# StavrosOrf/EV2Gym

Measured on AMD Instinct MI355X. Metric: env-steps/sec (envs x chargers x steps); % HBM roofline, higher is better.
Workload: dtype f64; 1 GPU; cfg2: V2GProfitPlusLoads, 50 chargers, 1 transformer, uniform[-1,1] actions; envs_per_gpu=4096, scenario_pool_per_gpu=32768, scenario_pool_order=sorted by busy window inside every window of envs_per_gpu scenarios, chargers=50, transformers=1, steps_per_episode=112, obs_dim=162, soc_log=True, launch=persistent, actor=none

## Files before the change

ev2gym_amd/csrc/ev2g_device.h:

```cpp
#pragma once
#include <hip/hip_runtime.h>
#include <stdint.h>

#define EV2G_BLOCK 256
#define EV2G_NQ 8

#include "ev2g_records.h"
typedef SessDyn PortDyn;

struct DevScn {
    int E;
    int M;
    int T, C, npc, P, R, D, ND, dt;
    int reward_kind, state_kind, flags, cost_kind;
    int n_lut;
    int G;
    int gs;
    int n_groups;
    double sixty_over_dt;
    double dt_over_60;
    const int *slot_port, *slot_cs, *slot_obs, *slot_tr;
    const int *cs_np, *cs_pbase, *slot_mask;
    const int *cs_slot0;
    int het;
// ... 854 lines not shown
    z = z ^ (z >> 31);
    return (double)(z >> 11) * (1.0 / 9007199254740992.0);
}

__global__ void ev2g_fill_uniform_kernel(double *dst, long long n, uint64_t seed, double lo, double hi) {
    for (long long i = blockIdx.x * (long long)blockDim.x + threadIdx.x; i < n; i += (long long)gridDim.x * blockDim.x)
        dst[i] = lo + (hi - lo) * ev2g_u01(seed, (uint64_t)i);
}

__device__ __forceinline__ double wave_sum(double v) {
    for (int d = 32; d > 0; d >>= 1) v += __shfl_xor(v, d, 64);
    return v;
}
__device__ __forceinline__ double wave_min(double v) {
    for (int d = 32; d > 0; d >>= 1) v = fmin(v, __shfl_xor(v, d, 64));
    return v;
}

__device__ __forceinline__ void port_sessions(const DevScn &s, const DevState &st, long long g, long long gs, int cur_step, int &first,
                                              int &last, bool &attached) {
    first = s.port_first[gs];
    last = first;
    attached = false;
    if (first < 0) return;
    const int2 w = make_int2(st.line[g].ta, st.line[g].td);
    const int cur = st.line[g].ss;
    if (cur < 0) {
        last = s.port_end[gs];
    } else {
        attached = (w.x <= cur_step);
        last = attached ? cur + 1 : cur;
    }
}

template <int EPWS> __device__ __forceinline__ double seg_sum(double v) {
    v += xor1_f64(v);
    v += xor2_f64(v);
    v += xor4_f64(v);
    v += dpp_mov_f64<0x128>(v);
    const int lo = __double2loint(v), hi = __double2hiint(v);
    const double r0 = __hiloint2double(__builtin_amdgcn_readlane(hi, 0), __builtin_amdgcn_readlane(lo, 0));
    const double r1 = __hiloint2double(__builtin_amdgcn_readlane(hi, 16), __builtin_amdgcn_readlane(lo, 16));
    const double r2 = __hiloint2double(__builtin_amdgcn_readlane(hi, 32), __builtin_amdgcn_readlane(lo, 32));
    const double r3 = __hiloint2double(__builtin_amdgcn_readlane(hi, 48), __builtin_amdgcn_readlane(lo, 48));
    if (EPWS == 1) return (r0 + r1) + (r2 + r3);
    return (threadIdx.x < 32) ? r0 + r1 : r2 + r3;
}
template <int EPWS> __device__ __forceinline__ double seg_min(double v) {
    v = fmin(v, xor1_f64(v));
    v = fmin(v, xor2_f64(v));
    v = fmin(v, xor4_f64(v));
    v = fmin(v, dpp_mov_f64<0x128>(v));
    const int lo = __double2loint(v), hi = __double2hiint(v);
    const double r0 = __hiloint2double(__builtin_amdgcn_readlane(hi, 0), __builtin_amdgcn_readlane(lo, 0));
    const double r1 = __hiloint2double(__builtin_amdgcn_readlane(hi, 16), __builtin_amdgcn_readlane(lo, 16));
    const double r2 = __hiloint2double(__builtin_amdgcn_readlane(hi, 32), __builtin_amdgcn_readlane(lo, 32));
    const double r3 = __hiloint2double(__builtin_amdgcn_readlane(hi, 48), __builtin_amdgcn_readlane(lo, 48));
    if (EPWS == 1) return fmin(fmin(r0, r1), fmin(r2, r3));
    return (threadIdx.x < 32) ? fmin(r0, r1) : fmin(r2, r3);
}
template <int EPWS> __device__ __forceinline__ bool seg_all(bool p) {
    const unsigned long long m = __ballot(p);
    if (EPWS == 1) return m == ~0ull;
    return (threadIdx.x < 32) ? ((unsigned)m == 0xffffffffu) : ((unsigned)(m >> 32) == 0xffffffffu);
}

struct StatsView {
    int T, C, R, P, dt;
    const double *setpoint;
    const int *scn_sess, *scn_sess_end, *ss_slot, *ss_tarr, *ss_tdep;
    const double *ss_B, *ss_afap;
    const int *cs_served;
    const double *cs_sat_sum, *hist, *env_acc, *sess_final_cap, *sess_abs_e, *soc_log;
    const PortLine *line;
};
__device__ __forceinline__ StatsView ev2g_stats_view(const DevScn &s, const DevState &st, const double *ss_afap) {
    return StatsView{s.T, s.C, s.R, s.P, s.dt, s.setpoint, s.scn_sess, s.scn_sess_end, s.ss_slot, s.ss_tarr, s.ss_tdep, s.ss_B, ss_afap,
                     st.cs_served, st.cs_sat_sum, st.hist, st.env_acc, st.sess_final_cap, st.sess_abs_e, st.soc_log, st.line};
}

#define EV2G_STATS_NK 40
#define EV2G_STATS_TB 8
#define EV2G_STATS_LK 16

template <int EPWS, int NK, int LK>
__device__ __forceinline__ void ev2g_env_stats(const StatsView &sv, int e, bool e_valid, int scn, int lane, int cur_step, double *__restrict__ out,
                                               double *l_keep, int lslot) {
    constexpr int W = 64 / EPWS;
    const int T = sv.T, C = sv.C, R = sv.R, P = sv.P;
    double served = 0.0, sat = 0.0, nsat = 0.0;
    for (int c = lane; c < C; c += W) {
        const int n = sv.cs_served[(long long)e * C + c];
        served += n;
        if (n > 0) { sat += sv.cs_sat_sum[(long long)e * C + c] / n; nsat += 1.0; }
    }
    served = seg_sum<EPWS>(served); sat = seg_sum<EPWS>(sat); nsat = seg_sum<EPWS>(nsat);
    double over = 0.0, te = 0.0, ete = 0.0, ptv = 0.0;
    for (int t = lane; t < T; t += W) {
        const bool past = t < cur_step;
        if (past) for (int r = 0; r < R; r++) over += sv.hist[EV2G_HIST(e, t, T, R) + 2 + r];
        const double sp = sv.setpoint[(long long)scn * T + t], u = past ? sv.hist[EV2G_HIST(e, t, T, R)] : 0.0;
        const double d = sp - u;
        te += d * d;
        ete += fabs(d);
        if (u > sp) ptv += u - sp;
    }
    over = seg_sum<EPWS>(over); te = seg_sum<EPWS>(te); ete = seg_sum<EPWS>(ete); ptv = seg_sum<EPWS>(ptv);
    ete *= (double)sv.dt / 60.0;
    if (lane == 0 && e_valid) {
        double *o = out + (long long)e * 17;
        o[0] = served;
        o[4] = (nsat > 0.0) ? sat / nsat : NAN;
        o[5] = ptv;
        o[6] = te;
        o[7] = ete;
        o[12] = over;
    }
    const double e0 = 7.543e6, e1 = 23.75e6, e2 = 6976, z0 = 7.348e-3, z1 = 3.667, z2 = 7.6e-4, z3 = 4.081e-3;
    const double b_cap_ah = 2.05, b_cap_kwh = 78, d_dist = 15000, b_age = 2 * 365, G_ = 0.186;
    const double theta = 298.15, kk = 0.8263, v_min = 3.3324;
    const double k_arrh = exp(-e2 / theta), k_age = pow(b_age, 0.25);
    const double Q_acc = 2 * (b_age * (d_dist / 365) * G_ * b_cap_ah) / b_cap_kwh, k_qacc = pow(Q_acc, 0.5);
    const bool log_soc = sv.soc_log != nullptr;
    double sum = 0.0, mn = INFINITY, cnt = 0.0, deg_cal = 0.0, deg_cyc = 0.0;
    double vkeep[2];
    int nkeep = 0;
    const int d0 = sv.scn_sess[scn], d1 = sv.scn_sess_end[scn];
    for (int k0 = d0; k0 < d1; k0 += W) {
        const int k = min(k0 + lane, d1 - 1);
        const bool has = k0 + lane < d1;
        const int q = sv.ss_slot[k], ta = sv.ss_tarr[k], td = sv.ss_tdep[k];
        const double B = sv.ss_B[k], afap = sv.ss_afap[k], fin_cap = sv.sess_final_cap[k];
        const double fin_abs = log_soc ? sv.sess_abs_e[k] : 0.0;
        const long long g = (long long)e * P + q;
        const bool spawned = has && ta <= cur_step;
        const bool live = td >= cur_step;
        const double l_cap = sv.line[g].cap, l_abs = sv.line[g].abse;
        const double capk = live ? l_cap : fin_cap;
        if (spawned) {
            const double v = capk / afap * 100.0;
            sum += v;
            mn = fmin(mn, v);
            cnt += 1.0;
            if (nkeep < 2) vkeep[nkeep] = v;
            nkeep++;
        }
        if (spawned) {
            if (log_soc) {
                const double *__restrict__ slog = sv.soc_log + (long long)e * T * P + q;
                const int tend = min(td, cur_step - 1);
                const double soc_f = capk / B;
                const double invB = 1.0 / B;
                double hs = 0.0, fs = 0.0;
                int n = 0, nf = 0;
                double xk[NK];
#pragma unroll
                for (int u = 0; u < NK; u++) xk[u] = slog[(long long)min(ta + u, tend) * P];
#pragma unroll
                for (int u = 0; u < NK; u++) {
                    if (ta + u <= tend) {
                        const double soc = fabs(xk[u]) * invB;
                        hs += soc; n++;
                        if (__double_as_longlong(xk[u]) >= 0) { fs += soc; nf++; }
                    }
                }
                for (int t = ta + NK; t <= tend; t += EV2G_STATS_TB) {
                    double x[EV2G_STATS_TB];
#pragma unroll
                    for (int u = 0; u < EV2G_STATS_TB; u++) x[u] = slog[(long long)min(t + u, tend) * P];
                    if (LK > 0 && t - ta - NK < LK) {
#pragma unroll
                        for (int u = 0; u < EV2G_STATS_TB; u++) l_keep[(t - ta - NK + u) * 64 + lslot] = x[u];
                    }
#pragma unroll
                    for (int u = 0; u < EV2G_STATS_TB; u++) {
                        if (t + u <= tend) {
                            const double soc = fabs(x[u]) * invB;
                            hs += soc; n++;
                            if (__double_as_longlong(x[u]) >= 0) { fs += soc; nf++; }
                        }
                    }
                }
                hs += soc_f; n++;
                fs += soc_f; nf++;
                const double avg_soc = hs / n, avg_f = fs / nf;
                double mad = 0.0;
#pragma unroll
                for (int u = 0; u < NK; u++)
                    if (ta + u <= tend && __double_as_longlong(xk[u]) >= 0) mad += fabs(avg_f - fabs(xk[u]) * invB);
                for (int t = ta + NK; t <= tend; t += EV2G_STATS_TB) {
                    double x[EV2G_STATS_TB];
                    if (LK > 0 && t - ta - NK < LK) {
#pragma unroll
                        for (int u = 0; u < EV2G_STATS_TB; u++) x[u] = l_keep[(t - ta - NK + u) * 64 + lslot];
                    } else {
#pragma unroll
                        for (int u = 0; u < EV2G_STATS_TB; u++) x[u] = slog[(long long)min(t + u, tend) * P];
                    }
#pragma unroll
                    for (int u = 0; u < EV2G_STATS_TB; u++)
                        if (t + u <= tend && __double_as_longlong(x[u]) >= 0) mad += fabs(avg_f - fabs(x[u]) * invB);
                }
                mad += fabs(avg_f - soc_f);
                const double delta_DoD = 2 * (mad / nf);
                const double T_sim = (td - ta + 1) * (double)sv.dt / (60 * 24);
                const double v_avg = v_min + kk * avg_soc;
                const double alpha = (e0 * v_avg - e1) * k_arrh;
                deg_cal += alpha * 0.75 * T_sim / k_age;
                const double v_half = v_min + kk * 0.5;
                const double beta = z0 * (v_half - z1) * (v_half - z1) + z2 + z3 * delta_DoD;
                const double abs_e = live ? l_abs : fin_abs;
                const double Q_sim = (abs_e / b_cap_kwh) * b_cap_ah;
                deg_cyc += beta * 0.5 * Q_sim / k_qacc;
            }
        }
    }
    sum = seg_sum<EPWS>(sum); cnt = seg_sum<EPWS>(cnt); mn = seg_min<EPWS>(mn);
    deg_cal = seg_sum<EPWS>(deg_cal); deg_cyc = seg_sum<EPWS>(deg_cyc);
    if (lane == 0 && e_valid) {
        const double *acc = sv.env_acc + (long long)e * 8;
        double *o = out + (long long)e * 17;
        o[1] = acc[1];
        o[2] = acc[2];
        o[3] = acc[3];
        o[11] = acc[4];
        o[13] = log_soc ? deg_cal + deg_cyc : NAN;
        o[14] = log_soc ? deg_cal : NAN;
        o[15] = log_soc ? deg_cyc : NAN;
        o[16] = acc[0];
    }
    double mean = NAN, sd = NAN, mnv = NAN;
    if (cnt > 0.0) {
        mean = sum / cnt;
        double var = 0.0;
        if (seg_all<EPWS>(nkeep <= 2)) {
            if (nkeep > 0) { const double v = vkeep[0] - mean; var += v * v; }
            if (nkeep > 1) { const double v = vkeep[1] - mean; var += v * v; }
        } else {
            for (int k = d0 + lane; k < d1; k += W) {
                const int ta = sv.ss_tarr[k];
                if (ta <= cur_step) {
                    const double capk = (sv.ss_tdep[k] >= cur_step) ? sv.line[(long long)e * P + sv.ss_slot[k]].cap : sv.sess_final_cap[k];
                    const double v = capk / sv.ss_afap[k] * 100.0 - mean;
                    var += v * v;
                }
            }
        }
        var = seg_sum<EPWS>(var);
        sd = sqrt(var / cnt);
        mnv = mn;
    }
    if (lane == 0 && e_valid) {
        double *o = out + (long long)e * 17;
        o[8] = mean;
        o[9] = sd;
        o[10] = mnv;
    }
}

template <int W>
__device__ __forceinline__ void ev2g_env_reset(const DevScn &s, const DevState &st, int e, int lane, int reset_off, double *__restrict__ r_obs,
                                               float *__restrict__ r_obs32) {
    const int T = s.T, C = s.C, R = s.R, P = s.P;
    const int scn_n = ev2g_scn(e, reset_off, s.M);
    const bool hfast = s.head_tab != nullptr && s.state_kind != 1 && 2 + s.head_nh <= 2 * W && (r_obs || r_obs32);
    double hrow0 = 0.0, hrow1 = 0.0;
    if (hfast) {
        const double *row = s.head_tab + (long long)scn_n * (T + 1) * s.head_nh;
        hrow0 = row[min(max(lane - 2, 0), s.head_nh - 1)];
        hrow1 = row[min(lane + W - 2, s.head_nh - 1)];
    }
    for (int q = lane; q < P; q += W) {
        const long long g = (long long)e * P + q, gs = (long long)scn_n * P + q;
        const int2 w = s.port_first_win[gs];
        st.line[g].ta = w.x; st.line[g].td = w.y; st.line[g].ss = s.port_first[gs]; st.line[g].cyc_lut = 0;
        st.line[g].cap = 0.0; st.line[g].tot = 0.0; st.line[g].prev = 0.0;
        st.port_energy[g] = 0.0; st.port_current[g] = 0.0;
        if (r_obs) { double *o = r_obs + (long long)e * s.D + s.slot_obs[q]; o[0] = 0.0; o[1] = 0.0; if (s.state_kind == 1) o[2] = 0.0; }
        if (r_obs32) { float *o = r_obs32 + (long long)e * s.D + s.slot_obs[q]; o[0] = 0.f; o[1] = 0.f; if (s.state_kind == 1) o[2] = 0.f; }
    }
    for (int c = lane; c < C; c += W) {
        const long long gc = (long long)e * C + c;
        st.cs_sat_sum[gc] = 0.0; st.cs_served[gc] = 0;
        if (st.cs_profits) { st.cs_profits[gc] = 0.0; st.cs_e_ch[gc] = 0.0; st.cs_e_dis[gc] = 0.0; st.cs_power_now[gc] = 0.0; st.cs_cur_now[gc] = 0.0; }
    }
    for (int i = lane; i < 8; i += W) st.env_acc[(long long)e * 8 + i] = 0.0;
    if (lane == 0) st.hist[EV2G_HIST(e, 0, T, R) + 1] = 0.0;
    for (int r = lane; r < R; r += W) st.tr_power_now[(long long)e * R + r] = 0.0;
    if (lane == 0) st.env_fault[e] = 0;
    if (hfast) {
        const int c0 = lane, c1 = lane + W, nc = 2 + s.head_nh;
        const double v0 = (c0 < 2) ? 0.0 : hrow0;
        if (r_obs) { double *o = r_obs + (long long)e * s.D; if (c0 < nc) o[c0] = v0; if (c1 < nc) o[c1] = hrow1; }
        if (r_obs32) { float *o = r_obs32 + (long long)e * s.D; if (c0 < nc) o[c0] = (float)v0; if (c1 < nc) o[c1] = (float)hrow1; }
    } else {
        if (r_obs) write_obs_env(s, r_obs + (long long)e * s.D, scn_n, 0, 0.0, lane, W);
        if (r_obs32) write_obs_env(s, r_obs32 + (long long)e * s.D, scn_n, 0, 0.0, lane, W);
    }
}

template <int EPWS, bool RESET = false>
__global__ void __launch_bounds__(64) ev2g_stats_kernel(DevScn s, DevState st, int scn_off,
                                                        const double *__restrict__ ss_afap, int cur_step,
                                                        double *__restrict__ out, int reset_off = 0, double *__restrict__ r_obs = nullptr,
                                                        float *__restrict__ r_obs32 = nullptr) {
    constexpr int W = 64 / EPWS;
    const int sub = threadIdx.x / W, lane = threadIdx.x - sub * W;
    const int e_raw = blockIdx.x * EPWS + sub;
    const bool e_valid = e_raw < s.E;
    const int e = e_valid ? e_raw : s.E - 1;
    const int scn = ev2g_scn(e, scn_off, s.M);
    extern __shared__ double l_keep[];
    ev2g_env_stats<EPWS, EV2G_STATS_NK, EV2G_STATS_LK>(ev2g_stats_view(s, st, ss_afap), e, e_valid, scn, lane, cur_step, out, l_keep, (int)threadIdx.x);
    if (RESET && e_valid) ev2g_env_reset<W>(s, st, e, lane, reset_off, r_obs, r_obs32);
}

template <int EPWS>
__global__ void __launch_bounds__(64) ev2g_copy_stats_reset_kernel(DevScn s, DevState st, const double *__restrict__ done_stats, double *__restrict__ out,
                                                                   int reset_off, double *__restrict__ r_obs, float *__restrict__ r_obs32) {
    constexpr int W = 64 / EPWS;
    const int sub = threadIdx.x / W, lane = threadIdx.x - sub * W;
    const int e = blockIdx.x * EPWS + sub;
    if (e >= s.E) return;
    for (int j = lane; j < 17; j += W) out[(long long)e * 17 + j] = done_stats[(long long)e * 17 + j];
    ev2g_env_reset<W>(s, st, e, lane, reset_off, r_obs, r_obs32);
}
```

ev2gym_amd/csrc/ev2g_host.hip:

```cpp
#include <hip/hip_runtime.h>

#include <algorithm>
#include <cmath>
#include <cstdio>
#include <cstring>
#include <array>
#include <map>
#include <string>
#include <utility>
#include <vector>

#include "../../include/ev2g.h"
#include "ev2g_device.h"
#include "ev2g_load_host.h"
#include "ev2g_route_host.h"
#include "ev2g_policy_host.h"
#include "ev2g_step_v2.h"
#include "ev2g_step_wave.h"
#include "ev2g_step_big.h"
#include "ev2g_mlp.h"
#include "ev2g_comm.h"
#include "ev2g_refill.h"
#include "ev2g_heuristic.h"
#include "ev2g_link.h"
// ... 2390 lines not shown
}

int ev2g_host_adam(float *theta, float *m, float *v, const float *g, int64_t n, int64_t t, double lr, double beta1, double beta2, double eps) {
    if (!theta || !m || !v || !g || n < 0 || t < 1) return fail(nullptr, EV2G_ERR_ARG, "ev2g_host_adam: null argument, n < 0 or t < 1");
    if (!std::isfinite(lr) || !(beta1 >= 0.0 && beta1 < 1.0) || !(beta2 >= 0.0 && beta2 < 1.0) || !(eps > 0.0))
        return fail(nullptr, EV2G_ERR_ARG, "ev2g_host_adam: lr must be finite, the betas in [0, 1), eps > 0");
    const AdamStep a = adam_step(lr, beta1, beta2, eps, (long long)t);
    for (int64_t i = 0; i < n; i++) ev2g_adam_elem(theta + i, m + i, v + i, g[i], a);
    return EV2G_OK;
}

int ev2g_host_ppo_head(const float *mean, const float *value, const float *actions, const float *log_std, const float *old_log_prob,
                       const float *advantages, const float *returns, int B, int P, const ev2g_ppo_config *cfg, float *d_mean, float *d_value,
                       float *d_log_std, float *stats) {
    if (!mean || !value || !actions || !log_std || !old_log_prob || !advantages || !returns || !cfg || !d_mean || !d_value || !d_log_std || !stats)
        return fail(nullptr, EV2G_ERR_ARG, "ev2g_host_ppo_head: null argument");
    if (B < 1 || P < 1) return fail(nullptr, EV2G_ERR_ARG, "ev2g_host_ppo_head: B and P must be positive");
    const bool norm = cfg->normalize_advantage && B > 1;
    double a_mean = 0.0, a_scale = 1.0;
    if (norm) {
        double s = 0.0;
        for (int i = 0; i < B; i++) s += (double)advantages[i];
        a_mean = s / B;
        s = 0.0;
        for (int i = 0; i < B; i++) { const double d = (double)advantages[i] - a_mean; s += d * d; }
        a_scale = 1.0 / (std::sqrt(s / (double)(B - 1)) + 1e-8);
    }
    std::vector<double> iv((size_t)P), dls((size_t)P, 0.0);
    for (int p = 0; p < P; p++) iv[(size_t)p] = std::exp(-2.0 * (double)log_std[p]);
    const double inv_b = 1.0 / (double)B;
    double sum[4] = {0.0, 0.0, 0.0, 0.0};
    for (int i = 0; i < B; i++) {
        const float *mu = mean + (size_t)i * P, *a = actions + (size_t)i * P;
        double q[8];
        for (int j = 0; j < 8; j++) q[j] = ev2g_ppo_lp_part(mu, a, log_std, iv.data(), P, j, 8);
        const float A = norm ? (float)(((double)advantages[i] - a_mean) * a_scale) : advantages[i];
        const PpoRow o = ev2g_ppo_head_row(ev2g_ppo_join8(q), old_log_prob[i], A, returns[i], value[i], (float)cfg->clip_range, (float)cfg->vf_coef, inv_b);
        d_value[i] = o.g_v;
        sum[0] += o.pol; sum[1] += o.vsq; sum[2] += o.kl; sum[3] += o.clipped;
        for (int p = 0; p < P; p++) {
            float dl;
            ev2g_ppo_head_port(a[p], mu[p], iv[(size_t)p], o.g_lp, d_mean + (size_t)i * P + p, &dl);
            dls[(size_t)p] += (double)dl;
        }
    }
    for (int p = 0; p < P; p++) d_log_std[p] = (float)(dls[(size_t)p] - cfg->ent_coef);
    ev2g_ppo_stats(sum, log_std, P, inv_b, (float)cfg->vf_coef, (float)cfg->ent_coef, stats);
    return EV2G_OK;
}

int ev2g_check_faults(ev2g_handle *h, int32_t *first_bad_env) {
    if (!h || !h->loaded) return fail(h, EV2G_ERR_STATE, "ev2g_check_faults: no scenarios loaded");
    (void)hipSetDevice(h->device);
    std::vector<int> f(h->E);
    HIPCHK(h, hipMemcpyAsync(f.data(), h->st.env_fault, sizeof(int) * h->E, hipMemcpyDeviceToHost, h->stream));
    HIPCHK(h, hipStreamSynchronize(h->stream));
    for (int e = 0; e < h->E; e++)
        if (f[e]) {
            if (first_bad_env) *first_bad_env = e;
            return fail(h, EV2G_ERR_OVERCURRENT, "charger over-current: sum of amps is higher than max charge current (ev_charger.py:203-205)");
        }
    return EV2G_OK;
}

static int launch_stats(ev2g_handle *h, double *stats, bool reset, double *obs, long long off, float *obs32 = nullptr) {
    (void)hipSetDevice(h->device);
    const bool copy = h->last.inl_stats && h->current_step == h->T;
    h->last_stats_route = copy ? 1 : 0;
    h->stats_reason = copy ? "" : h->last.inl_reason;
    if (copy && !reset) {
        HIPCHK(h, hipMemcpyAsync(stats, h->d_stats_inl, sizeof(double) * (size_t)h->E * EV2G_N_STATS, hipMemcpyDeviceToDevice, h->stream));
        return EV2G_OK;
    }

    const bool pair = stats_pair(h);
    const dim3 grid(pair ? (h->E + 1) / 2 : h->E);
    if (copy) {
        hipLaunchKernelGGL((ev2g_copy_stats_reset_kernel<1>), dim3(h->E), dim3(64), 0, h->stream, h->scn, h->st, (const double *)h->d_stats_inl, stats, (int)off, obs,
                           obs32 ? obs32 : (float *)h->extras.obs_f32);
        HIPCHK(h, hipGetLastError());
        return EV2G_OK;
    }
#define EV2G_STATS_LAUNCH(EPWS, RESET)                                                                                                    \
    hipLaunchKernelGGL((ev2g_stats_kernel<EPWS, RESET>), grid, dim3(64), (size_t)EV2G_STATS_LK * 64 * sizeof(double), h->stream, h->scn, h->st, (int)h->scn_off, (const double *)h->d_ss_afap, \
                       h->current_step, stats, (int)off, obs, RESET ? (obs32 ? obs32 : (float *)h->extras.obs_f32) : (float *)nullptr)
    if (pair) { if (reset) EV2G_STATS_LAUNCH(2, true); else EV2G_STATS_LAUNCH(2, false); }
    else { if (reset) EV2G_STATS_LAUNCH(1, true); else EV2G_STATS_LAUNCH(1, false); }
#undef EV2G_STATS_LAUNCH
    HIPCHK(h, hipGetLastError());
    return EV2G_OK;
}

int ev2g_get_stats(ev2g_handle *h, double *stats) {
    if (!h || !h->loaded) return fail(h, EV2G_ERR_STATE, "ev2g_get_stats: no scenarios loaded");
    if (!stats) return fail(h, EV2G_ERR_ARG, "ev2g_get_stats: null output");
    return launch_stats(h, stats, false, nullptr, 0);
}

static int stats_reset_impl(ev2g_handle *h, double *stats, double *obs, float *obs32, int64_t scenario_offset) {
    if (!h || !h->loaded) return fail(h, EV2G_ERR_STATE, "ev2g_get_stats_reset: no scenarios loaded");
    if (!stats) return fail(h, EV2G_ERR_ARG, "ev2g_get_stats_reset: null output");
    long long off = scenario_offset % (long long)h->scn.M;
    if (off < 0) off += h->scn.M;
    const int rc = launch_stats(h, stats, true, obs, off, obs32);
    if (rc) return rc;
    if (h->st.cs_power_hist) {
        HIPCHK(h, hipMemsetAsync(h->st.cs_power_hist, 0, sizeof(double) * (size_t)h->scn.T * h->scn.E * h->scn.C, h->stream));
        HIPCHK(h, hipMemsetAsync(h->st.cs_cur_hist, 0, sizeof(double) * (size_t)h->scn.T * h->scn.E * h->scn.C, h->stream));
    }
    h->scn_off = off;
    h->current_step = 0;
    state_changed(h, "the episode was reset");
    return EV2G_OK;
}
int ev2g_get_stats_reset(ev2g_handle *h, double *stats, double *obs, int64_t scenario_offset) { return stats_reset_impl(h, stats, obs, nullptr, scenario_offset); }
int ev2g_get_stats_reset_f32(ev2g_handle *h, double *stats, float *obs32, int64_t scenario_offset) { return stats_reset_impl(h, stats, nullptr, obs32, scenario_offset); }

int ev2g_comm_get_unique_id(void *id) {
    RcclApi *api = rccl_api();
    if (!api->lib) return fail(nullptr, EV2G_ERR_STATE, "ev2g_comm_get_unique_id: " + api->err);
    if (!id) return fail(nullptr, EV2G_ERR_ARG, "ev2g_comm_get_unique_id: null output");
    static_assert(sizeof(ncclUniqueId) == EV2G_COMM_ID_BYTES, "EV2G_COMM_ID_BYTES must be sizeof(ncclUniqueId)");
    ncclUniqueId u;
    const ncclResult_t r = api->GetUniqueId(&u);
    if (r != ncclSuccess) return fail(nullptr, EV2G_ERR_HIP, std::string("ncclGetUniqueId: ") + api->GetErrorString(r));
    std::memcpy(id, &u, sizeof u);
    return EV2G_OK;
}

int ev2g_comm_init(ev2g_handle *h, const void *id, int rank, int world_size) {
    if (!h) return fail(h, EV2G_ERR_ARG, "ev2g_comm_init: null handle");
    if (!id || world_size < 1 || rank < 0 || rank >= world_size) return fail(h, EV2G_ERR_ARG, "ev2g_comm_init: bad arguments");
    RcclApi *api = rccl_api();
    if (!api->lib) return fail(h, EV2G_ERR_STATE, "ev2g_comm_init: " + api->err);
    ev2g_comm_destroy(h);
    (void)hipSetDevice(h->device);
    ncclUniqueId u;
    std::memcpy(&u, id, sizeof u);
    const ncclResult_t r = api->CommInitRank(&h->comm.comm, world_size, u, rank);
    if (r != ncclSuccess) { h->comm.comm = nullptr; return fail(h, EV2G_ERR_HIP, std::string("ncclCommInitRank: ") + api->GetErrorString(r)); }
    h->comm.rank = rank; h->comm.world = world_size;
    return EV2G_OK;
}

void ev2g_comm_destroy(ev2g_handle *h) {
    if (!h || !h->comm.comm) return;
    (void)hipSetDevice(h->device);
    (void)hipStreamSynchronize(h->stream);
    rccl_api()->CommDestroy(h->comm.comm);
    if (h->comm.d_send) (void)hipFree(h->comm.d_send);
    h->comm = CommState{};
}

int ev2g_comm_world_size(const ev2g_handle *h) { return (h && h->comm.comm) ? h->comm.world : 0; }
long long ev2g_comm_gathers(const ev2g_handle *h) { return h ? h->comm.gathers : 0; }

int ev2g_gather_stats(ev2g_handle *h, double *stats_all) {
    if (!h || !h->loaded) return fail(h, EV2G_ERR_STATE, "ev2g_gather_stats: no scenarios loaded");
    if (!h->comm.comm) return fail(h, EV2G_ERR_STATE, "ev2g_gather_stats: no communicator (call ev2g_comm_init on every rank first)");
    if (!stats_all) return fail(h, EV2G_ERR_ARG, "ev2g_gather_stats: null output");
    (void)hipSetDevice(h->device);
    if (h->comm.send_envs != h->E) {
        if (h->comm.d_send) { (void)hipStreamSynchronize(h->stream); (void)hipFree(h->comm.d_send); h->comm.d_send = nullptr; }
        HIPCHK(h, hipMalloc((void **)&h->comm.d_send, sizeof(double) * (size_t)h->E * EV2G_N_STATS));
        h->comm.send_envs = h->E;
    }
    RcclApi *api = rccl_api();
// ... 225 lines not shown
```

ev2gym_amd/csrc/ev2g_step_wave.h:

```cpp
#pragma once
#include <type_traits>
#include "ev2g_step_v2.h"
#include "ev2g_mlp.h"

#define EV2G_WAVE_BLOCK 256
#ifndef EV2G_FF_N_MIN
#define EV2G_FF_N_MIN 1
#endif

__host__ __device__ inline size_t ev2g_wave_lds_bytes(int envs_per_group, int block = EV2G_WAVE_BLOCK) {
    const size_t NS = (size_t)block;
    return sizeof(double) * (EV2G_NQ * (NS + 8) + 7 * NS + 7 * (size_t)envs_per_group + 4 * 64) + sizeof(int) * (6 * NS + 8);
}
#define EV2G_INL_STATS_NK 12
#define EV2G_INL_STATS_LK 16
__host__ __device__ inline size_t ev2g_inl_stats_lds_bytes(int block = EV2G_WAVE_BLOCK) { return (size_t)block * EV2G_INL_STATS_LK * sizeof(double); }
#define EV2G_FUSED_BLOCK 1024
#define EV2G_FUSED_SX 200
#define EV2G_FUSED_RING 10
#define EV2G_FUSED_RING2 7

#define EV2G_FUSED_SXF 196
#define EV2G_FUSED_RINGF 4
__host__ __device__ inline size_t ev2g_fused_lds_bytes(int envs_per_wave = 1, int weight_terms = 1) {
    if (weight_terms > 1)
        return ev2g_wave_lds_bytes(EV2G_FUSED_BLOCK / 64 * envs_per_wave, EV2G_FUSED_BLOCK) + (size_t)16 * EV2G_FUSED_SXF * 4;
    return ev2g_wave_lds_bytes(EV2G_FUSED_BLOCK / 64 * envs_per_wave, EV2G_FUSED_BLOCK) + (size_t)16 * EV2G_FUSED_SX * 2 + (size_t)(25 + 19 + 4) * 16 * 4;
}
struct FusedArgs {
    MlpDev m;
    const float *obs0;
};

typedef const char __attribute__((address_space(1))) *gcptr;
typedef char __attribute__((address_space(1))) *gptr;
template <class T, class B> __device__ __forceinline__ T ldg32(B base, unsigned boff) {
    return *(const T __attribute__((address_space(1))) *)((gcptr)base + boff);
}
template <class T, class B> __device__ __forceinline__ T ldg32_nt(B base, unsigned boff) {
    return __builtin_nontemporal_load((const T __attribute__((address_space(1))) *)((gcptr)base + boff));
}
template <class T, class B> __device__ __forceinline__ void stg32(B base, unsigned boff, T v) {
    *(T __attribute__((address_space(1))) *)((gptr)base + boff) = v;
}
template <class T, class B> __device__ __forceinline__ void stg32_nt(B base, unsigned boff, T v) {
    __builtin_nontemporal_store(v, (T __attribute__((address_space(1))) *)((gptr)base + boff));
}
typedef double d2v __attribute__((ext_vector_type(2)));
typedef double d2v_a8 __attribute__((ext_vector_type(2), aligned(8)));
typedef int i2v __attribute__((ext_vector_type(2)));
typedef int i4v __attribute__((ext_vector_type(4)));
typedef float f2v __attribute__((ext_vector_type(2)));
template <class B> __device__ __forceinline__ SessRec ldg32_rec_charge(B base, unsigned boff) {
    union { SessRec r; d2v v[sizeof(SessRec) / 16]; } u;
    static_assert(sizeof(SessRec) == 128 && offsetof(SessRec, rB) == 48 && offsetof(SessRec, rv) == 64 && offsetof(SessRec, minB) == 80 && offsetof(SessRec, cap0) == 112,
                  "charging reads chunks 0..4, discharging chunks 3..6");
#pragma unroll
    for (int i = 0; i < 5; i++) u.v[i] = ldg32<d2v>(base, boff + 16u * i);
    asm volatile("" : "+v"(u.v[0]), "+v"(u.v[1]), "+v"(u.v[2]), "+v"(u.v[3]), "+v"(u.v[4]));
    return u.r;
}
template <class B> __device__ __forceinline__ SessRec ldg32_rec_discharge(B base, unsigned boff) {
    union { SessRec r; d2v v[sizeof(SessRec) / 16]; } u;
#pragma unroll
    for (int i = 3; i < 7; i++) u.v[i] = ldg32<d2v>(base, boff + 16u * i);
    asm volatile("" : "+v"(u.v[3]), "+v"(u.v[4]), "+v"(u.v[5]), "+v"(u.v[6]));
    return u.r;
}

template <class B> __device__ __forceinline__ SessRec ldg32_cls_charge(B base, unsigned boff) {
    static_assert(sizeof(ClsRec) == 128 && offsetof(ClsRec, gate_ch) == 16 && offsetof(ClsRec, rB) == 32 && offsetof(ClsRec, rv) == 48 && offsetof(ClsRec, v_d) == 64 &&
                  offsetof(ClsRec, gate_dis) == 80 && offsetof(ClsRec, emerg) == 96, "ClsRec layout");
    d2v c[4];
#pragma unroll
    for (int i = 0; i < 4; i++) c[i] = ldg32<d2v>(base, boff + 16u * i);
    asm volatile("" : "+v"(c[0]), "+v"(c[1]), "+v"(c[2]), "+v"(c[3]));
    SessRec r;
    r.pacmax = c[0].x; r.tsm = c[0].y; r.gate_ch = c[1].x; r.B = c[1].y; r.rB = c[2].x; r.v = c[2].y; r.rv = c[3].x;
    return r;
}
template <class B> __device__ __forceinline__ SessRec ldg32_cls_discharge(B base, unsigned boff) {
    d2v c[3];
#pragma unroll
    for (int i = 0; i < 3; i++) c[i] = ldg32<d2v>(base, boff + 64u + 16u * i);
    asm volatile("" : "+v"(c[0]), "+v"(c[1]), "+v"(c[2]));
    SessRec r;
    r.v = c[0].x; r.rv = c[0].y; r.gate_dis = c[1].x; r.minB = c[1].y; r.emerg = c[2].x; r.pdismax = c[2].y;
    return r;
}

struct WaveArgs {
    int P, T, E, D, M;
    char *slab_port; unsigned long long slab_port_slice;
    double *hist;
    double *env_acc;
    const double *cs_pack;
    char *lines;
    const double *step_tab;
    char *port_dyn;
// ... 764 lines not shown
                }
            }
        }
        if ((valid || hcopy) && ((F32 && out) || (!FULL && obs32))) {
            const unsigned o4 = FULL ? hb_obs_env : (unsigned)(e_l * D) * 4u;
            if (SK == 1) {
                if (q_l == 0) {
                    const float h0 = (float)((double)sstep / (double)T), h1 = (float)((sstep < T) ? pf_ob0 : 0.0), h2 = (float)usage;
                    stg32<float>(obs32, o4, h0);
                    stg32<float>(obs32, o4 + 4u, h1);
                    stg32<float>(obs32, o4 + 8u, h2);
                    if (ACT && NWF > 1) { bufXf[arow * FSXF] = h0; bufXf[arow * FSXF + 1] = h1; bufXf[arow * FSXF + 2] = h2; }
                    else
                    if (ACT) {
                        *(uint32_t *)(bufX + arow * FSX) = ev2g_pack_bf16(h0, h1);
                        bufX[arow * FSX + 2] = (uint16_t)ev2g_pack_bf16(h2, 0.f);
                    }
                }
            } else {
                if (q_l == 0) stg32<f2v>(obs32, o4, (f2v){(float)sstep, (float)usage});
                if (q_l < NPAIR) stg32<f2v>(obs32, o4 + 8u + (unsigned)q_l * 8u, (f2v){(float)pf_h0.x, (float)pf_h0.y});
                if (ACT) {
                    if (q_l == 0) xput2(0, (float)sstep, (float)usage);
                    if (q_l < NPAIR) xput2(2 + 2 * q_l, (float)pf_h0.x, (float)pf_h0.y);
                }
                if (!WIDE) {
                    if (q_l + P < NPAIR) stg32<f2v>(obs32, o4 + 8u + (unsigned)(q_l + P) * 8u, (f2v){(float)pf_h1.x, (float)pf_h1.y});
                    const unsigned h8 = (unsigned)((scn * (T + 1) + sstep) * NHEAD) * 8u;
                    for (int pi = q_l + 2 * P; pi < NPAIR; pi += P) {
                        const d2v hv = ldg32<d2v>(S->head_tab, h8 + (unsigned)pi * 16u);
                        stg32<f2v>(obs32, o4 + 8u + (unsigned)pi * 8u, (f2v){(float)hv.x, (float)hv.y});
                    }
                }
            }
        }
        if (valid && ((F64 && out) || (!FULL && obs))) {
            const unsigned o8 = FULL ? hb_obs_env : (unsigned)(e_l * D) * 8u;
            if (SK == 1) {
                if (q_l == 0) {
                    stg32<double>(obs, o8, (double)sstep / (double)T);
                    stg32<double>(obs, o8 + 8u, (sstep < T) ? pf_ob0 : 0.0);
                    stg32<double>(obs, o8 + 16u, usage);
                }
            } else {
                if (STR_NT) {
                    if (q_l == 0) stg32_nt<d2v>(obs, o8, (d2v){(double)sstep, usage});
                    if (q_l < NPAIR) stg32_nt<d2v>(obs, o8 + 16u + (unsigned)q_l * 16u, pf_h0);
                } else {
                if (q_l == 0) stg32<d2v>(obs, o8, (d2v){(double)sstep, usage});
                if (q_l < NPAIR) stg32<d2v>(obs, o8 + 16u + (unsigned)q_l * 16u, pf_h0);
                }
                if (!WIDE) {
                    if (q_l + P < NPAIR) stg32<d2v>(obs, o8 + 16u + (unsigned)(q_l + P) * 16u, pf_h1);
                    const unsigned h8 = (unsigned)((scn * (T + 1) + sstep) * NHEAD) * 8u;
                    for (int pi = q_l + 2 * P; pi < NPAIR; pi += P)
                        stg32<d2v>(obs, o8 + 16u + (unsigned)pi * 16u, ldg32<d2v>(S->head_tab, h8 + (unsigned)pi * 16u));
                }
            }
        }
        PT_MARK(5)
        PT_STEP_END(cntk[0] + cntk[1] == 0)
        t += 1;
        if (STR) { obs_run += io.o_stride; rew_run += io.r_stride; done_run += io.d_stride; mask_run += io.m_stride; }
        if (ACT) obs32_run += io.o_stride;
    }
    __syncthreads();
    if (valid) {
        const int d = s_dirty[tid];
        const unsigned g8 = (unsigned)g * 8u;
        if (d & 3) stg32<i4v>(wa.lines, l64, (i4v){FULL ? r_ta : s_ta[tid], FULL ? r_td : s_td[tid], s_ss[tid], ev2g_line_pack(s_cyc[tid], ((d >> 8) & LUTMASK) - 1)});
        if (d & 1) {
            stg32<d2v>(wa.lines, l64 + 16u, (d2v){s_cap[tid], s_tot[tid]});
            stg32<d2v>(wa.lines, l64 + 32u, (d2v){s_prev[tid], s_abse[tid]});
        }
    }
#if defined(EV2G_PHASE_TIMING) && defined(EV2G_PT_OUTER)
    asm volatile("s_waitcnt vmcnt(0)" ::: "memory");
    PT_MARK(6)
#endif
    PT_FLUSH
    double *stats_out = (INL && t == T && k_steps > 1) ? (double *)S->stats_inl : nullptr;
    if (stats_out != nullptr) {
        __syncthreads();
        const int es = e0 + wv;
        if (es < S->E) {
            const int scn_s = (int)(__builtin_amdgcn_readfirstlane(hb_step) / (64u * (unsigned)T));
            StatsView v{T, S->C, S->R, P, S->dt, (const double *)S->setpoint, (const int *)S->scn_sess, (const int *)S->scn_sess_end,
                        (const int *)S->ss_slot, (const int *)S->ss_tarr, (const int *)S->ss_tdep, (const double *)S->ss_B, (const double *)S->ss_afap,
                        (const int *)S->cs_served, (const double *)S->cs_sat_sum, (const double *)S->hist, (const double *)S->env_acc,
                        (const double *)S->sess_final_cap, (const double *)S->sess_abs_e, (const double *)S->soc_log, (const PortLine *)S->line};
            ev2g_env_stats<1, EV2G_INL_STATS_NK, EV2G_INL_STATS_LK>(v, es, true, scn_s, lane, T, stats_out,
                                                                  lds + (size_t)wv * EV2G_INL_STATS_LK * 64, lane);
        }
    }
}
```

Baseline: 1.227 billion env-steps/s.

## Prefetch stats inputs up front and software-pipeline soc_log reads in env stats

```diff
diff --git a/ev2gym_amd/csrc/ev2g_device.h b/ev2gym_amd/csrc/ev2g_device.h
--- a/ev2gym_amd/csrc/ev2g_device.h
+++ b/ev2gym_amd/csrc/ev2g_device.h
@@ -960,29 +960,64 @@
 #define EV2G_STATS_NK 40
 #define EV2G_STATS_TB 8
 #define EV2G_STATS_LK 16
-
-template <int EPWS, int NK, int LK>
+#define EV2G_STATS_RB 8
+__host__ __device__ constexpr size_t ev2g_stats_lds_doubles(int lk) { return (size_t)(lk + 3) * 64; }
+
+struct StatsSess {
+    int q, ta, td;
+    double B, afap, fin_cap, fin_abs;
+};
+__device__ __forceinline__ StatsSess ev2g_stats_sess(const StatsView &sv, int k, bool log_soc) {
+    return StatsSess{sv.ss_slot[k], sv.ss_tarr[k], sv.ss_tdep[k], sv.ss_B[k], sv.ss_afap[k], sv.sess_final_cap[k], log_soc ? sv.sess_abs_e[k] : 0.0};
+}
+
+template <int EPWS, int NK, int LK, int TB>
 __device__ __forceinline__ void ev2g_env_stats(const StatsView &sv, int e, bool e_valid, int scn, int lane, int cur_step, double *__restrict__ out,
                                                double *l_keep, int lslot) {
-    constexpr int W = 64 / EPWS;
+    constexpr int W = 64 / EPWS, RB = EV2G_STATS_RB;
+    static_assert(TB % RB == 0 && LK % RB == 0, "the second pass walks the LDS block and the re-read range in whole batches of RB");
     const int T = sv.T, C = sv.C, R = sv.R, P = sv.P;
+    const bool log_soc = sv.soc_log != nullptr;
+    if (EPWS == 1) e = __builtin_amdgcn_readfirstlane(e);
+    const int d0 = sv.scn_sess[scn], d1 = sv.scn_sess_end[scn];
+    const int c_0 = min(lane, C - 1);
+    const int n_0 = sv.cs_served[(long long)e * C + c_0];
+    const double ss_0 = sv.cs_sat_sum[(long long)e * C + c_0];
+    const int t_0 = min(lane, T - 1), t_1 = min(lane + W, T - 1);
+    const double hu_0 = sv.hist[EV2G_HIST(e, t_0, T, R)], hu_1 = sv.hist[EV2G_HIST(e, t_1, T, R)];
+    const double ho_0 = (R > 0) ? sv.hist[EV2G_HIST(e, t_0, T, R) + 2] : 0.0, ho_1 = (R > 0) ? sv.hist[EV2G_HIST(e, t_1, T, R) + 2] : 0.0;
+    const double sp_0 = sv.setpoint[(long long)scn * T + t_0], sp_1 = sv.setpoint[(long long)scn * T + t_1];
+    const double acc_l = sv.env_acc[(long long)e * 8 + min(lane, 7)];
+    StatsSess ss{0, 0, 0, 1.0, 1.0, 0.0, 0.0};
+    if (d0 < d1) ss = ev2g_stats_sess(sv, min(d0 + lane, d1 - 1), log_soc);
     double served = 0.0, sat = 0.0, nsat = 0.0;
-    for (int c = lane; c < C; c += W) {
+    if (lane < C) {
+        served += n_0;
+        if (n_0 > 0) { sat += ss_0 / n_0; nsat += 1.0; }
+    }
+    for (int c = lane + W; c < C; c += W) {
         const int n = sv.cs_served[(long long)e * C + c];
         served += n;
         if (n > 0) { sat += sv.cs_sat_sum[(long long)e * C + c] / n; nsat += 1.0; }
     }
     served = seg_sum<EPWS>(served); sat = seg_sum<EPWS>(sat); nsat = seg_sum<EPWS>(nsat);
     double over = 0.0, te = 0.0, ete = 0.0, ptv = 0.0;
-    for (int t = lane; t < T; t += W) {
+    auto hist_step = [&](int t, double hu, double ho, double sp) {
         const bool past = t < cur_step;
-        if (past) for (int r = 0; r < R; r++) over += sv.hist[EV2G_HIST(e, t, T, R) + 2 + r];
-        const double sp = sv.setpoint[(long long)scn * T + t], u = past ? sv.hist[EV2G_HIST(e, t, T, R)] : 0.0;
+        if (past) {
+            over += ho;
+            for (int r = 1; r < R; r++) over += sv.hist[EV2G_HIST(e, t, T, R) + 2 + r];
+        }
+        const double u = past ? hu : 0.0;
         const double d = sp - u;
         te += d * d;
         ete += fabs(d);
         if (u > sp) ptv += u - sp;
-    }
+    };
+    if (lane < T) hist_step(lane, hu_0, ho_0, sp_0);
+    if (lane + W < T) hist_step(lane + W, hu_1, ho_1, sp_1);
+    for (int t = lane + 2 * W; t < T; t += W)
+        hist_step(t, sv.hist[EV2G_HIST(e, t, T, R)], (R > 0) ? sv.hist[EV2G_HIST(e, t, T, R) + 2] : 0.0, sv.setpoint[(long long)scn * T + t]);
     over = seg_sum<EPWS>(over); te = seg_sum<EPWS>(te); ete = seg_sum<EPWS>(ete); ptv = seg_sum<EPWS>(ptv);
     ete *= (double)sv.dt / 60.0;
     if (lane == 0 && e_valid) {
@@ -994,126 +1029,157 @@
         o[7] = ete;
         o[12] = over;
     }
+    if (lane < 5 && e_valid) {
+        const int col = (lane == 0) ? 16 : (lane == 4) ? 11 : lane;
+        out[(long long)e * 17 + col] = acc_l;
+    }
     const double e0 = 7.543e6, e1 = 23.75e6, e2 = 6976, z0 = 7.348e-3, z1 = 3.667, z2 = 7.6e-4, z3 = 4.081e-3;
     const double b_cap_ah = 2.05, b_cap_kwh = 78, d_dist = 15000, b_age = 2 * 365, G_ = 0.186;
     const double theta = 298.15, kk = 0.8263, v_min = 3.3324;
     const double k_arrh = exp(-e2 / theta), k_age = pow(b_age, 0.25);
     const double Q_acc = 2 * (b_age * (d_dist / 365) * G_ * b_cap_ah) / b_cap_kwh, k_qacc = pow(Q_acc, 0.5);
-    const bool log_soc = sv.soc_log != nullptr;
     double sum = 0.0, mn = INFINITY, cnt = 0.0, deg_cal = 0.0, deg_cyc = 0.0;
-    double vkeep[2];
     int nkeep = 0;
-    const int d0 = sv.scn_sess[scn], d1 = sv.scn_sess_end[scn];
+    double *l_vkeep = l_keep + (size_t)LK * 64 + lslot;
     for (int k0 = d0; k0 < d1; k0 += W) {
-        const int k = min(k0 + lane, d1 - 1);
         const bool has = k0 + lane < d1;
-        const int q = sv.ss_slot[k], ta = sv.ss_tarr[k], td = sv.ss_tdep[k];
-        const double B = sv.ss_B[k], afap = sv.ss_afap[k], fin_cap = sv.sess_final_cap[k];
-        const double fin_abs = log_soc ? sv.sess_abs_e[k] : 0.0;
+        const int q = ss.q, ta = ss.ta, td = ss.td;
+        const double B = ss.B, afap = ss.afap, fin_cap = ss.fin_cap, fin_abs = ss.fin_abs;
         const long long g = (long long)e * P + q;
         const bool spawned = has && ta <= cur_step;
         const bool live = td >= cur_step;
         const double l_cap = sv.line[g].cap, l_abs = sv.line[g].abse;
+        const int tend = min(td, cur_step - 1);
+        const int len = tend - ta;
+        const int tclamp = max(tend, 0), r0 = min(ta, tclamp);
+        const int lenc = tclamp - r0;
+        typedef const char __attribute__((address_space(1))) *log_base_t;
+        log_base_t lbase = nullptr;
+        const double *__restrict__ slog = nullptr;
+        if (log_soc) {
+            if (EPWS == 1) {
+                lbase = (log_base_t)(sv.soc_log + (long long)e * T * P);
+            } else {
+                slog = sv.soc_log + ((long long)e * T + r0) * P + q;
+            }
+        }
+        const unsigned P8 = (unsigned)P * 8u, off0 = (unsigned)r0 * P8 + (unsigned)q * 8u;
+        auto log_entry = [&](int j) -> double {
+            if (EPWS == 1) return *(const double __attribute__((address_space(1))) *)(lbase + (off0 + (unsigned)j * P8));
+            return slog[(long long)j * P];
+        };
         const double capk = live ? l_cap : fin_cap;
-        if (spawned) {
-            const double v = capk / afap * 100.0;
-            sum += v;
-            mn = fmin(mn, v);
-            cnt += 1.0;
-            if (nkeep < 2) vkeep[nkeep] = v;
-            nkeep++;
-        }
-        if (spawned) {
-            if (log_soc) {
-                const double *__restrict__ slog = sv.soc_log + (long long)e * T * P + q;
-                const int tend = min(td, cur_step - 1);
+        auto satisfaction = [&]() {
+            if (spawned) {
+                const double v = capk / afap * 100.0;
+                sum += v;
+                mn = fmin(mn, v);
+                cnt += 1.0;
+                if (nkeep < 2) l_vkeep[nkeep * 64] = v;
+                nkeep++;
+            }
+        };
+        if (log_soc) {
+            double xk[NK], xb[TB];
+#pragma unroll
+            for (int u = 0; u < NK; u++) xk[u] = log_entry(min(u, lenc));
+#pragma unroll
+            for (int u = 0; u < TB; u++) xb[u] = log_entry(min(NK + u, lenc));
+            satisfaction();
+            if (spawned) {
+                l_vkeep[2 * 64] = live ? l_abs : fin_abs;
+                const int dur = td - ta + 1;
                 const double soc_f = capk / B;
                 const double invB = 1.0 / B;
                 double hs = 0.0, fs = 0.0;
-                int n = 0, nf = 0;
-                double xk[NK];
-#pragma unroll
-                for (int u = 0; u < NK; u++) xk[u] = slog[(long long)min(ta + u, tend) * P];
+                int nf = 0;
 #pragma unroll
                 for (int u = 0; u < NK; u++) {
-                    if (ta + u <= tend) {
+                    if (u <= len) {
                         const double soc = fabs(xk[u]) * invB;
-                        hs += soc; n++;
+                        hs += soc;
                         if (__double_as_longlong(xk[u]) >= 0) { fs += soc; nf++; }
                     }
                 }
-                for (int t = ta + NK; t <= tend; t += EV2G_STATS_TB) {
-                    double x[EV2G_STATS_TB];
-#pragma unroll
-                    for (int u = 0; u < EV2G_STATS_TB; u++) x[u] = slog[(long long)min(t + u, tend) * P];
-                    if (LK > 0 && t - ta - NK < LK) {
-#pragma unroll
-                        for (int u = 0; u < EV2G_STATS_TB; u++) l_keep[(t - ta - NK + u) * 64 + lslot] = x[u];
+                int bo = 0, rem = len - NK;
+                while (rem >= 0) {
+                    const bool more = rem >= TB;
+                    if (LK > 0 && more && bo < LK) {
+#pragma unroll
+                        for (int u = 0; u < TB; u++)
+                            if (LK % TB == 0 || bo + u < LK) l_keep[(bo + u) * 64 + lslot] = xb[u];
                     }
 #pragma unroll
-                    for (int u = 0; u < EV2G_STATS_TB; u++) {
-                        if (t + u <= tend) {
-                            const double soc = fabs(x[u]) * invB;
-                            hs += soc; n++;
-                            if (__double_as_longlong(x[u]) >= 0) { fs += soc; nf++; }
+                    for (int u = 0; u < TB; u++) {
+                        if (u <= rem) {
+                            const double soc = fabs(xb[u]) * invB;
+                            hs += soc;
+                            if (__double_as_longlong(xb[u]) >= 0) { fs += soc; nf++; }
                         }
                     }
+                    if (!more) break;
+                    bo += TB; rem -= TB;
+#pragma unroll
+                    for (int u = 0; u < TB; u++) xb[u] = log_entry(NK + bo + min(u, rem));
                 }
-                hs += soc_f; n++;
+                const int n = len + 2;
+                hs += soc_f;
                 fs += soc_f; nf++;
                 const double avg_soc = hs / n, avg_f = fs / nf;
                 double mad = 0.0;
 #pragma unroll
                 for (int u = 0; u < NK; u++)
-                    if (ta + u <= tend && __double_as_longlong(xk[u]) >= 0) mad += fabs(avg_f - fabs(xk[u]) * invB);
-                for (int t = ta + NK; t <= tend; t += EV2G_STATS_TB) {
-                    double x[EV2G_STATS_TB];
-                    if (LK > 0 && t - ta - NK < LK) {
-#pragma unroll
-                        for (int u = 0; u < EV2G_STATS_TB; u++) x[u] = l_keep[(t - ta - NK + u) * 64 + lslot];
+                    if (u <= len && __double_as_longlong(xk[u]) >= 0) mad += fabs(avg_f - fabs(xk[u]) * invB);
+                for (int b2 = 0; b2 < bo; b2 += RB) {
+                    double x[RB];
+                    if (LK > 0 && b2 < LK) {
+#pragma unroll
+                        for (int u = 0; u < RB; u++) x[u] = l_keep[(b2 + u) * 64 + lslot];
                     } else {
 #pragma unroll
-                        for (int u = 0; u < EV2G_STATS_TB; u++) x[u] = slog[(long long)min(t + u, tend) * P];
+                        for (int u = 0; u < RB; u++) x[u] = log_entry(NK + b2 + u);
                     }
 #pragma unroll
-                    for (int u = 0; u < EV2G_STATS_TB; u++)
-                        if (t + u <= tend && __double_as_longlong(x[u]) >= 0) mad += fabs(avg_f - fabs(x[u]) * invB);
+                    for (int u = 0; u < RB; u++)
+                        if (__double_as_longlong(x[u]) >= 0) mad += fabs(avg_f - fabs(x[u]) * invB);
                 }
+#pragma unroll
+                for (int u = 0; u < TB; u++)
+                    if (u <= rem && __double_as_longlong(xb[u]) >= 0) mad += fabs(avg_f - fabs(xb[u]) * invB);
                 mad += fabs(avg_f - soc_f);
                 const double delta_DoD = 2 * (mad / nf);
-                const double T_sim = (td - ta + 1) * (double)sv.dt / (60 * 24);
+                int dt_s = sv.dt;
+                asm volatile("" : "+s"(dt_s));
+                const double T_sim = dur * (double)dt_s / (60 * 24);
                 const double v_avg = v_min + kk * avg_soc;
                 const double alpha = (e0 * v_avg - e1) * k_arrh;
                 deg_cal += alpha * 0.75 * T_sim / k_age;
                 const double v_half = v_min + kk * 0.5;
                 const double beta = z0 * (v_half - z1) * (v_half - z1) + z2 + z3 * delta_DoD;
-                const double abs_e = live ? l_abs : fin_abs;
+                const double abs_e = l_vkeep[2 * 64];
                 const double Q_sim = (abs_e / b_cap_kwh) * b_cap_ah;
                 deg_cyc += beta * 0.5 * Q_sim / k_qacc;
             }
-        }
+        } else {
+            satisfaction();
+        }
+        if (k0 + W < d1) ss = ev2g_stats_sess(sv, min(k0 + W + lane, d1 - 1), log_soc);
     }
     sum = seg_sum<EPWS>(sum); cnt = seg_sum<EPWS>(cnt); mn = seg_min<EPWS>(mn);
     deg_cal = seg_sum<EPWS>(deg_cal); deg_cyc = seg_sum<EPWS>(deg_cyc);
     if (lane == 0 && e_valid) {
-        const double *acc = sv.env_acc + (long long)e * 8;
         double *o = out + (long long)e * 17;
-        o[1] = acc[1];
-        o[2] = acc[2];
-        o[3] = acc[3];
-        o[11] = acc[4];
         o[13] = log_soc ? deg_cal + deg_cyc : NAN;
         o[14] = log_soc ? deg_cal : NAN;
         o[15] = log_soc ? deg_cyc : NAN;
-        o[16] = acc[0];
     }
     double mean = NAN, sd = NAN, mnv = NAN;
     if (cnt > 0.0) {
         mean = sum / cnt;
         double var = 0.0;
         if (seg_all<EPWS>(nkeep <= 2)) {
-            if (nkeep > 0) { const double v = vkeep[0] - mean; var += v * v; }
-            if (nkeep > 1) { const double v = vkeep[1] - mean; var += v * v; }
+            if (nkeep > 0) { const double v = l_vkeep[0] - mean; var += v * v; }
+            if (nkeep > 1) { const double v = l_vkeep[64] - mean; var += v * v; }
         } else {
             for (int k = d0 + lane; k < d1; k += W) {
                 const int ta = sv.ss_tarr[k];
@@ -1189,7 +1255,7 @@
     const int e = e_valid ? e_raw : s.E - 1;
     const int scn = ev2g_scn(e, scn_off, s.M);
     extern __shared__ double l_keep[];
-    ev2g_env_stats<EPWS, EV2G_STATS_NK, EV2G_STATS_LK>(ev2g_stats_view(s, st, ss_afap), e, e_valid, scn, lane, cur_step, out, l_keep, (int)threadIdx.x);
+    ev2g_env_stats<EPWS, EV2G_STATS_NK, EV2G_STATS_LK, EV2G_STATS_TB>(ev2g_stats_view(s, st, ss_afap), e, e_valid, scn, lane, cur_step, out, l_keep, (int)threadIdx.x);
     if (RESET && e_valid) ev2g_env_reset<W>(s, st, e, lane, reset_off, r_obs, r_obs32);
 }
 
diff --git a/ev2gym_amd/csrc/ev2g_host.hip b/ev2gym_amd/csrc/ev2g_host.hip
--- a/ev2gym_amd/csrc/ev2g_host.hip
+++ b/ev2gym_amd/csrc/ev2g_host.hip
@@ -2496,7 +2496,7 @@
         return EV2G_OK;
     }
 #define EV2G_STATS_LAUNCH(EPWS, RESET)                                                                                                    \
-    hipLaunchKernelGGL((ev2g_stats_kernel<EPWS, RESET>), grid, dim3(64), (size_t)EV2G_STATS_LK * 64 * sizeof(double), h->stream, h->scn, h->st, (int)h->scn_off, (const double *)h->d_ss_afap, \
+    hipLaunchKernelGGL((ev2g_stats_kernel<EPWS, RESET>), grid, dim3(64), ev2g_stats_lds_doubles(EV2G_STATS_LK) * sizeof(double), h->stream, h->scn, h->st, (int)h->scn_off, (const double *)h->d_ss_afap, \
                        h->current_step, stats, (int)off, obs, RESET ? (obs32 ? obs32 : (float *)h->extras.obs_f32) : (float *)nullptr)
     if (pair) { if (reset) EV2G_STATS_LAUNCH(2, true); else EV2G_STATS_LAUNCH(2, false); }
     else { if (reset) EV2G_STATS_LAUNCH(1, true); else EV2G_STATS_LAUNCH(1, false); }
diff --git a/ev2gym_amd/csrc/ev2g_step_wave.h b/ev2gym_amd/csrc/ev2g_step_wave.h
--- a/ev2gym_amd/csrc/ev2g_step_wave.h
+++ b/ev2gym_amd/csrc/ev2g_step_wave.h
@@ -12,9 +12,14 @@
     const size_t NS = (size_t)block;
     return sizeof(double) * (EV2G_NQ * (NS + 8) + 7 * NS + 7 * (size_t)envs_per_group + 4 * 64) + sizeof(int) * (6 * NS + 8);
 }
+#ifndef EV2G_INL_STATS_NK
 #define EV2G_INL_STATS_NK 12
+#endif
+#ifndef EV2G_INL_STATS_TB
+#define EV2G_INL_STATS_TB 8
+#endif
 #define EV2G_INL_STATS_LK 16
-__host__ __device__ inline size_t ev2g_inl_stats_lds_bytes(int block = EV2G_WAVE_BLOCK) { return (size_t)block * EV2G_INL_STATS_LK * sizeof(double); }
+__host__ __device__ inline size_t ev2g_inl_stats_lds_bytes(int block = EV2G_WAVE_BLOCK) { return (size_t)(block / 64) * ev2g_stats_lds_doubles(EV2G_INL_STATS_LK) * sizeof(double); }
 #define EV2G_FUSED_BLOCK 1024
 #define EV2G_FUSED_SX 200
 #define EV2G_FUSED_RING 10
@@ -945,15 +950,18 @@
     double *stats_out = (INL && t == T && k_steps > 1) ? (double *)S->stats_inl : nullptr;
     if (stats_out != nullptr) {
         __syncthreads();
-        const int es = e0 + wv;
+        int tid_s = tid;
+        asm volatile("" : "+v"(tid_s));
+        const int wv_s = tid_s >> 6;
+        const int es = e0 + wv_s;
         if (es < S->E) {
             const int scn_s = (int)(__builtin_amdgcn_readfirstlane(hb_step) / (64u * (unsigned)T));
             StatsView v{T, S->C, S->R, P, S->dt, (const double *)S->setpoint, (const int *)S->scn_sess, (const int *)S->scn_sess_end,
                         (const int *)S->ss_slot, (const int *)S->ss_tarr, (const int *)S->ss_tdep, (const double *)S->ss_B, (const double *)S->ss_afap,
                         (const int *)S->cs_served, (const double *)S->cs_sat_sum, (const double *)S->hist, (const double *)S->env_acc,
                         (const double *)S->sess_final_cap, (const double *)S->sess_abs_e, (const double *)S->soc_log, (const PortLine *)S->line};
-            ev2g_env_stats<1, EV2G_INL_STATS_NK, EV2G_INL_STATS_LK>(v, es, true, scn_s, lane, T, stats_out,
-                                                                  lds + (size_t)wv * EV2G_INL_STATS_LK * 64, lane);
+            ev2g_env_stats<1, EV2G_INL_STATS_NK, EV2G_INL_STATS_LK, EV2G_INL_STATS_TB>(v, es, true, scn_s, lane, T, stats_out,
+                                                                                     lds + (size_t)wv_s * ev2g_stats_lds_doubles(EV2G_INL_STATS_LK), lane);
         }
     }
 }
```

Result: no change. 1.232 billion env-steps/s, median of 6 (+0.4%).
